# Wang-Ruocheng/QuanONet

Measured on AMD Instinct MI355X. Metric: train samples/sec (circuit-evals/sec alongside), QuanONet Q=5 Net40-2-20-2 Advection, higher is better.
Workload: dtype f64

## Files before the change

### quanonet_amd/csrc/hea_inst.hip

```cpp
#include "hea_device.hpp"
#include "hea_zyz.hpp"
#include "hea_qsweep.hpp"

#ifndef QHEA_N
#error "compile with -DQHEA_N=<qubits>"
#endif
#define QHEA_CAT_(a, b) a##b
#define QHEA_CAT(a, b) QHEA_CAT_(a, b)

namespace qhea {

void QHEA_CAT(launch_fwd_, QHEA_N)(dim3 grid, hipStream_t st, const FwdArgs& a) {
    hipLaunchKernelGGL(fwd_kernel<QHEA_N>, grid, dim3(kWaves * 64), 0, st, a.runs, a.B, a.E, a.cs, a.gates, a.gates_bytes, a.off,
                       a.co, a.diag, a.pauli, a.out, a.state_out, a.bias);
}
void QHEA_CAT(launch_bwd_, QHEA_N)(dim3 grid, hipStream_t st, const BwdArgs& a) {
#if QHEA_N == 8 || QHEA_N == 9
    if (a.dense) {
        hipLaunchKernelGGL((bwd_kernel<QHEA_N, 2>), grid, dim3(kWaves * 64), 0, st, a.runs, a.B, a.E, a.blk, a.cs, a.gates,
                           a.gates_bytes, a.off, a.co, a.diag, a.pauli, a.g, a.state_in, a.y, a.bias, a.inv_bt, a.out,
                           a.grad_x, a.partial);
        return;
    }
#endif
// ... 15 lines not shown
                       a.partial, DepthArgs{mrec, ms});
}

void QHEA_CAT(launch_bwd_qubit_, QHEA_N)(dim3 grid, hipStream_t st, const BwdArgs& a, const QubitArgs& q) {
#if QHEA_N >= 7
#if QHEA_N == 8 || QHEA_N == 9
    if (a.dense) {
        hipLaunchKernelGGL((bwd_kernel<QHEA_N, 2, QubitArgs>), grid, dim3(kWaves * 64), 0, st, a.runs, a.B, a.E, a.blk, a.cs, a.gates,
                           a.gates_bytes, a.off, a.co, a.diag, a.pauli, a.g, a.state_in, a.y, a.bias, a.inv_bt, a.out,
                           a.grad_x, a.partial, q);
        return;
    }
#endif
    hipLaunchKernelGGL((bwd_kernel<QHEA_N, 1, QubitArgs>), grid, dim3(kWaves * 64), 0, st, a.runs, a.B, a.E, a.blk, a.cs, a.gates,
                       a.gates_bytes, a.off, a.co, a.diag, a.pauli, a.g, a.state_in, a.y, a.bias, a.inv_bt, a.out, a.grad_x,
                       a.partial, q);
#else
    (void)grid; (void)st; (void)a; (void)q;
#endif
}

void QHEA_CAT(launch_bwd_pair_, QHEA_N)(dim3 grid, hipStream_t st, const BwdArgs& a) {
#if QHEA_N <= 5
    if (a.tri == 1) {
        hipLaunchKernelGGL(bwd_tri_kernel<QHEA_N>, grid, dim3(128 + 64 * kSigmaWaves), 0, st, a.runs, a.B, a.E, a.blk, a.cs, a.gates,
                           a.gates_bytes, a.off, a.co, a.diag, a.pauli, a.g, a.state_in, a.y, a.bias, a.inv_bt, a.out,
                           a.grad_x, a.partial, a.status);
        return;
    }
    hipLaunchKernelGGL(bwd_pair_kernel<QHEA_N>, grid, dim3(128), 0, st, a.runs, a.B, a.E, a.blk, a.cs, a.gates,
                       a.gates_bytes, a.off, a.co, a.diag, a.pauli, a.g, a.state_in, a.y, a.bias, a.inv_bt, a.out, a.grad_x,
                       a.partial, a.status);
#else
    (void)grid; (void)st; (void)a;
#endif
}

#if QHEA_N <= 5
void QHEA_CAT(launch_fwd_zyz_, QHEA_N)(dim3 grid, size_t dyn_lds, hipStream_t st, const ZFwdArgs& a) {
    hipLaunchKernelGGL(fwd_zyz_kernel<QHEA_N>, grid, dim3((kZFwdWaves + kFwdHelpers) * 64), dyn_lds, st, a);
}
void QHEA_CAT(launch_bwd_ztri_, QHEA_N)(dim3 grid, size_t dyn_lds, hipStream_t st, const ZBwdArgs& a, const char* mrec) {
    if (grid.y > 1) {
        const ZBwdArgsM am{a, mrec};
        if (a.pipes == 2) hipLaunchKernelGGL((bwd_ztri_kernel<QHEA_N, 2, ZBwdArgsM>), grid, dim3(2 * 64 * kZPipeWaves), dyn_lds, st, am);
        else hipLaunchKernelGGL((bwd_ztri_kernel<QHEA_N, 1, ZBwdArgsM>), grid, dim3(64 * kZPipeWaves), dyn_lds, st, am);
        return;
    }
    if (a.pipes == 2) hipLaunchKernelGGL((bwd_ztri_kernel<QHEA_N, 2>), grid, dim3(2 * 64 * kZPipeWaves), dyn_lds, st, a);
    else hipLaunchKernelGGL((bwd_ztri_kernel<QHEA_N, 1>), grid, dim3(64 * kZPipeWaves), dyn_lds, st, a);
}
void QHEA_CAT(launch_fwd_zshared_, QHEA_N)(dim3 grid, size_t dyn_lds, hipStream_t st, const ZFwdArgs& a) {
    hipLaunchKernelGGL(fwd_zshared_kernel<QHEA_N>, grid, dim3(kZPWaves * 64), dyn_lds, st, a);
}
void QHEA_CAT(launch_bwd_zpacked_, QHEA_N)(dim3 grid, size_t dyn_lds, hipStream_t st, const ZBwdArgs& a, const char* mrec) {
    if (grid.y > 1) hipLaunchKernelGGL((bwd_zpacked_kernel<QHEA_N, ZBwdArgsM>), grid, dim3(kZPWaves * 64), dyn_lds, st, ZBwdArgsM{a, mrec});
    else hipLaunchKernelGGL(bwd_zpacked_kernel<QHEA_N>, grid, dim3(kZPWaves * 64), dyn_lds, st, a);
}
#if QHEA_N == 5
void launch_fwd_split_5(dim3 grid, size_t dyn_lds, hipStream_t st, const ZFwdArgs& a) {
    hipLaunchKernelGGL(fwd_split_kernel<5>, grid, dim3((kSplitWaves + kSplitHelpers) * 64), dyn_lds, st, a);
}
void launch_bwd_zquad_5(dim3 grid, size_t dyn_lds, hipStream_t st, const ZBwdArgs& a, const char* mrec) {
    if (grid.y > 1) hipLaunchKernelGGL((bwd_zquad_kernel<kPairRing, kZSigma, ZBwdArgsM>), grid, dim3(64 * (4 + kZSigma)), dyn_lds, st, ZBwdArgsM{a, mrec});
    else hipLaunchKernelGGL((bwd_zquad_kernel<kPairRing, kZSigma>), grid, dim3(64 * (4 + kZSigma)), dyn_lds, st, a);
}
void launch_bwd_zsnap_5(dim3 grid, size_t dyn_lds, hipStream_t st, const ZBwdArgs& a) {
    hipLaunchKernelGGL((bwd_zsnap_kernel<kZSnapRing>), grid, dim3(64 * (4 + 2 * kZSigma)), dyn_lds, st, a);
}
#endif
#elif QHEA_N <= 5
void QHEA_CAT(launch_fwd_zyz_, QHEA_N)(dim3, size_t, hipStream_t, const ZFwdArgs&) {}
void QHEA_CAT(launch_bwd_ztri_, QHEA_N)(dim3, size_t, hipStream_t, const ZBwdArgs&, const char*) {}
void QHEA_CAT(launch_bwd_zpacked_, QHEA_N)(dim3, size_t, hipStream_t, const ZBwdArgs&, const char*) {}
void QHEA_CAT(launch_fwd_zshared_, QHEA_N)(dim3, size_t, hipStream_t, const ZFwdArgs&) {}
#if QHEA_N == 5
void launch_fwd_split_5(dim3, size_t, hipStream_t, const ZFwdArgs&) {}
void launch_bwd_zquad_5(dim3, size_t, hipStream_t, const ZBwdArgs&, const char*) {}
void launch_bwd_zsnap_5(dim3, size_t, hipStream_t, const ZBwdArgs&) {}
#endif
#endif

}
```

### quanonet_amd/csrc/hea_zyz.hpp

```cpp
#pragma once
#include "hea_device.hpp"
#include "hea_sincos.hpp"

namespace qhea {

constexpr int kRecBytes = 1024;
constexpr int kRecRy = 512;
constexpr int kZCsBytes = 20480;

__host__ __device__ inline long zyz_cs_row(int n, long E) { return E + 2 * n; }
__host__ __device__ inline bool zyz_eligible(int n, long E) {
    return n >= 2 && n <= 5 && (long)(64 >> n) * zyz_cs_row(n, E) * 16 <= kZCsBytes;
}
__host__ __device__ inline int zyz_layer_count(const Runs& r, int n) {
    long L = 0;
    for (int i = 0; i < r.nruns; ++i) L += (long)r.count[i] * ((r.enc[i] + n - 1) / n + r.ld[i]);
    return (int)L;
}

struct AngleSrc {
    const double* x;
    EncDesc enc;
    long m_rows = 0, m_params = 0;
};
// ... 129 lines not shown
        const int lc = l < 0 ? 0 : (l > L ? L : l);
        dma_record(rsrc, lds0 + (unsigned)(l & (kSlots - 1)) * kRecBytes, lane16, (unsigned)lc * kRecBytes);
    }
    __device__ __forceinline__ char* buf(int l) const { return ring + (l & (kSlots - 1)) * kRecBytes; }
    __device__ __forceinline__ double2 rd_diag(int l) const { return *reinterpret_cast<const double2*>(buf(l) + dgoff); }
    template <int Q>
    __device__ __forceinline__ double2 rd_ry(int l) const { return *reinterpret_cast<const double2*>(buf(l) + voff[Q]); }
    __device__ __forceinline__ void rd_all_ry(int l) { static_for<0, N>([&](auto q) { ry[decltype(q)::value] = rd_ry<decltype(q)::value>(l); }); }

    template <int D>
    __device__ __forceinline__ void prime(int l0) {
#pragma unroll
        for (int i = 0; i < kDist; ++i) issue(l0 + i * D);
        wait_vmcnt<kDist - 1>();
        dg = rd_diag(l0);
        rd_all_ry(l0);
    }
    template <int D>
    __device__ __forceinline__ void begin(int l) {
        issue(l + kDist * D);
        wait_vmcnt<kDist - 1>();
    }
};

template <int N>
__device__ __forceinline__ void zyz_forward(double (&re)[1], double (&im)[1], const Runs& runs, LayerStream<N>& ls,
                                            const double2* __restrict__ csrow, int E, int lane, int klow, int ring_fwd) {
    re[0] = klow == 0 ? 1.0 : 0.0;
    im[0] = 0.0;
    int l = 0, col = 0;
    ls.template prime<1>(0);
    double2 nxt[N];
    auto prefetch = [&](int c) {
        static_for<0, N>([&](auto q) {
            constexpr int Q = decltype(q)::value;
            const int e = c + Q;
            nxt[Q] = csrow[e < E ? e : (E > 0 ? E - 1 : 0)];
        });
    };
    if (E > 0) prefetch(0);
    for (int ri = 0; ri < runs.nruns; ++ri) {
        const int ne = runs.enc[ri], nld = runs.ld[ri];
        for (int rep = 0; rep < runs.count[ri]; ++rep) {
            for (int j0 = 0; j0 < ne; j0 += N) {
                const int m = (ne - j0) < N ? (ne - j0) : N;
                ls.template begin<1>(l);
                apply_phase<false>(re[0], im[0], ls.dg);
                ls.dg = ls.rd_diag(l + 1);
                for_gates_below<N>(m, [&](auto q) {
                    constexpr int Q = decltype(q)::value;
                    apply_enc<N, Q, false>(re, im, nxt[Q]);
                });
                prefetch(col + j0 + m);
                ls.rd_all_ry(l + 1);
                ++l;
            }
            col += ne;
            for (int s = 0; s < nld; ++s) {
                ls.template begin<1>(l);
                apply_phase<false>(re[0], im[0], ls.dg);
                ls.dg = ls.rd_diag(l + 1);
                static_for<0, N>([&](auto q) {
                    constexpr int Q = decltype(q)::value;
                    apply_ry<Q, false>(re[0], im[0], ls.ry[Q]);
                    ls.ry[Q] = ls.template rd_ry<Q>(l + 1);
                });
                re[0] = lane_gather(re[0], ring_fwd);
                im[0] = lane_gather(im[0], ring_fwd);
                ++l;
            }
        }
    }
    apply_phase<false>(re[0], im[0], ls.dg);
}

template <int K> using CtSlot = std::integral_constant<int, K>;
struct RtSlot { int b; };
template <class T> struct is_ct_slot : std::false_type {};
template <int K> struct is_ct_slot<CtSlot<K>> : std::true_type {};
constexpr int kBSlots = 4, kBDist = 2;
constexpr int kPadRecs = 9;
constexpr int kBlockRingBytes = kBSlots * 3 * kRecBytes;

template <int N, int LD, bool SHARED = false>
struct BlockStream {
    static constexpr int RPB = 1 + LD;
    bool loader = true;
    u32x4 rsrc;
    char* ring;
    unsigned lds0, lane16, a_dg;
    unsigned a_ry[N];
    double2 dg[RPB];
    double2 ry[LD][N];
    double2 cs[N];

    __device__ __forceinline__ void init(const char* rec0, int nrec , char* ring_wave, int lane, int klow) {
        const unsigned long long base = reinterpret_cast<unsigned long long>(rec0) - (unsigned long long)kPadRecs * kRecBytes;
        rsrc = u32x4{(unsigned)base, (unsigned)(base >> 32) & 0xffffu, (unsigned)((nrec + 2 * kPadRecs) * kRecBytes), 0x00020000u};
        ring = ring_wave;
        lds0 = (unsigned)(unsigned long long)(__attribute__((address_space(3))) char*)ring_wave;
        lane16 = (unsigned)lane * 16u;
        a_dg = (unsigned)klow * 16u;
        static_for<0, N>([&](auto q) {
            constexpr int Q = decltype(q)::value;
            a_ry[Q] = kRecRy + Q * 32 + (Q == 4 ? 1u : (((unsigned)lane >> Q) & 1u)) * 16u;
        });
    }
    __device__ __forceinline__ void issue(int b) const {
        const unsigned slot = lds0 + (unsigned)(b & (kBSlots - 1)) * (RPB * kRecBytes);
        const unsigned soff = (unsigned)((b * RPB + kPadRecs) * kRecBytes);
        dma_records<RPB>(rsrc, slot, lane16, soff);
    }
    __device__ __forceinline__ const char* slot(int b) const { return ring + (b & (kBSlots - 1)) * (RPB * kRecBytes); }
    template <int D, int K>
    static constexpr int slot_off(CtSlot<K>) { return ((K + D) & (kBSlots - 1)) * (RPB * kRecBytes); }
    template <int D>
    static __device__ __forceinline__ int slot_off(RtSlot s) { return ((s.b + D) & (kBSlots - 1)) * (RPB * kRecBytes); }
    template <int D, class SL>
    __device__ __forceinline__ const char* slot_rel(SL s) const { return ring + slot_off<D>(s); }
    template <int D, class SL>
    __device__ __forceinline__ void ahead_rel(SL s, int b) const {
        if (!SHARED || loader)
            dma_records<RPB>(rsrc, lds0 + (unsigned)slot_off<D>(s), lane16, (unsigned)(((b + D) * RPB + kPadRecs) * kRecBytes));
    }
    __device__ __forceinline__ void landed() const {
        if (!SHARED || loader) wait_vmcnt<(kBDist - 1) * RPB>();
        if constexpr (SHARED) __syncthreads();
    }
    __device__ __forceinline__ void landed_late() const {
        if (!SHARED || loader) wait_vmcnt<kBDist * RPB>();
        if constexpr (SHARED) __syncthreads();
    }
    template <int D>
    __device__ __forceinline__ void ahead(int b) const { if (!SHARED || loader) issue(b + (kBDist + 1) * D); }
    template <int D>
    __device__ __forceinline__ void step(int b) const {
        ahead<D>(b);
        if (!SHARED || loader) wait_vmcnt<kBDist * RPB>();
        if constexpr (SHARED) __syncthreads();
    }
    template <int D>
    __device__ __forceinline__ void prime(int b0, bool drain) const {
        if (!SHARED || loader) {
            if (drain) wait_vmcnt<0>();
        }
        if constexpr (SHARED) { if (drain) __syncthreads(); }
        if (!SHARED || loader) {
#pragma unroll
            for (int i = 0; i <= kBDist; ++i) issue(b0 + i * D);
            wait_vmcnt<kBDist * RPB>();
        }
        if constexpr (SHARED) __syncthreads();
    }
    static __device__ __forceinline__ double2 rd(const char* p, unsigned off) { return *reinterpret_cast<const double2*>(p + off); }
    __device__ __forceinline__ void load_records(const char* sl) {
#pragma unroll
        for (int i = 0; i < RPB; ++i) dg[i] = rd(sl, i * kRecBytes + a_dg);
#pragma unroll
        for (int s = 0; s < LD; ++s)
            static_for<0, N>([&](auto q) { ry[s][decltype(q)::value] = rd(sl, (1 + s) * kRecBytes + a_ry[decltype(q)::value]); });
    }
    __device__ __forceinline__ void load_cs(const double2* __restrict__ csrow, int c0) {
        const double2* p = csrow + c0;
        static_for<0, N>([&](auto q) { cs[decltype(q)::value] = p[decltype(q)::value]; });
    }
};
// ... 93 lines not shown
    }
}
template <int Q>
__device__ __forceinline__ double2 cs32_packed(const double2* chunk ) {
    if constexpr (Q == 4) { const double2 t = chunk[2 * Q]; return make_double2(t.y, t.x); }
    else return chunk[2 * Q + 1];
}

template <bool HALVES>
__device__ __forceinline__ void swap_dup(double x, double& A, double& B) {
    double y;
    asm("" : "=v"(y) : "0"(x));
    const unsigned lo = (unsigned)__double2loint(x), hi = (unsigned)__double2hiint(x);
    const unsigned lo2 = (unsigned)__double2loint(y), hi2 = (unsigned)__double2hiint(y);
    if constexpr (HALVES) {
        const auto l = __builtin_amdgcn_permlane32_swap(lo, lo2, false, false);
        const auto h = __builtin_amdgcn_permlane32_swap(hi, hi2, false, false);
        A = __hiloint2double((int)h[0], (int)l[0]); B = __hiloint2double((int)h[1], (int)l[1]);
    } else {
        const auto l = __builtin_amdgcn_permlane16_swap(lo, lo2, false, false);
        const auto h = __builtin_amdgcn_permlane16_swap(hi, hi2, false, false);
        A = __hiloint2double((int)h[0], (int)l[0]); B = __hiloint2double((int)h[1], (int)l[1]);
    }
}
__device__ __forceinline__ void split_phase(double& x, const double2& d ) {
    double A, B;
    swap_dup<true>(x, A, B);
    x = d.y * A + d.x * B;
}
template <int Q>
__device__ __forceinline__ void split_ry(double& x, const double2& u) {
    if constexpr (Q == 4) {
        double A, B;
        swap_dup<false>(x, A, B);
        x = u.x * A + u.y * B;
    } else {
        const double own = u.x * x;
        x = fma(u.y, xchg<(1 << Q)>(x), own);
    }
}
struct SplitCoef { double2 dg; double t[4]; double2 g4; };
template <int Q>
__device__ __forceinline__ void split_ry_tan(double& x, double t) {
    static_assert(Q < 4, "wire 4 keeps the swap form");
    x = fma(t, xchg<(1 << Q)>(x), x);
}
__device__ __forceinline__ void split_gates(double& x, const LayerCoef<5>& c) {
    static_for<0, 5>([&](auto q) { split_ry<decltype(q)::value>(x, c.g[decltype(q)::value]); });
}
__device__ __forceinline__ void split_gates(double& x, const SplitCoef& c) {
    static_for<0, 4>([&](auto q) { split_ry_tan<decltype(q)::value>(x, c.t[decltype(q)::value]); });
    split_ry<4>(x, c.g4);
}

template <int LD>
struct SplitStream : BlockStream<5, LD, false> {
    using Base = BlockStream<5, LD, false>;
    static constexpr int RPB = 1 + LD;
    unsigned a_cs[5];
    __device__ __forceinline__ void init_split(const char* srec0, int nrec, char* ring_wave, int lane) {
        Base::init(srec0, nrec, ring_wave, lane, lane & 31);
        this->a_dg = (unsigned)(lane & 31) * 24u + (unsigned)(lane >> 5) * 8u;
        static_for<0, 5>([&](auto q) {
            constexpr int Q = decltype(q)::value;
            const unsigned bit = ((unsigned)lane >> Q) & 1u;
            this->a_ry[Q] = Q == 4 ? kSRecRy + 64 + bit * 16u : kSRecRy + Q * 16 + bit * 8u;
            a_cs[Q] = Q * 32 + (Q == 4 ? (1u - bit) : bit) * 16u;
        });
    }
    static __device__ __forceinline__ double2 rd8(const char* p, unsigned off) {
        const double* q = reinterpret_cast<const double*>(p + off);
        return make_double2(q[0], q[1]);
    }
    template <bool DAG = false>
    __device__ __forceinline__ void read_ansatz(SplitCoef& c, const char* sl, int rec, unsigned a_diag) const {
        c.dg = rd8(sl, rec * kRecBytes + a_diag);
        static_for<0, 4>([&](auto q) {
            constexpr int Q = decltype(q)::value;
            c.t[Q] = *reinterpret_cast<const double*>(sl + rec * kRecBytes + (this->a_ry[Q] ^ (DAG ? 8u : 0u)));
        });
        c.g4 = Base::rd(sl, rec * kRecBytes + this->a_ry[4]);
    }
};

constexpr int kSnapBytes = 1024;
template <int LD, bool SNAP = false>
__device__ __forceinline__ double zsplit_forward(SplitStream<LD>& bs, const char* csrow, int nblocks, int lane, int ring_fwd,
                                                 char* snap_base = nullptr, unsigned snap_off = 0) {
    double x = lane == 0 ? 1.0 : 0.0;
    bs.template prime<1>(0, false);
    const char* cs_b = csrow;
    LayerCoef<5> ce;
    SplitCoef ca, cb;
    ce.dg = bs.rd8(bs.slot(0), bs.a_dg);
    static_for<0, 5>([&](auto q) { ce.g[decltype(q)::value] = bs.rd(cs_b, bs.a_cs[decltype(q)::value]); });
    auto read_layer = [&](SplitCoef& c, const char* sl, int rec) {
        bs.read_ansatz(c, sl, rec, bs.a_dg);
        __builtin_amdgcn_sched_barrier(0);
    };
    auto read_chunk = [&](const char* nx, int kb) {
        ce.dg = bs.rd8(nx, bs.a_dg);
        const char* cn = cs_b + (kb + 1) * (5 * 32);
        static_for<0, 5>([&](auto q) { ce.g[decltype(q)::value] = bs.rd(cn, bs.a_cs[decltype(q)::value]); });
        __builtin_amdgcn_sched_barrier(0);
    };
    auto layer = [&](const auto& c, bool ring, int pt) {
        split_phase(x, c.dg);
        split_gates(x, c);
        if constexpr (SNAP) {
            if (ring) {
                typedef __attribute__((address_space(1))) double gdouble;
                *(gdouble*)(snap_base + (size_t)(unsigned)pt * kSnapBytes + snap_off) = x;
            }
        }
        __builtin_amdgcn_sched_barrier(0);
        if (ring) x = lane_gather(x, ring_fwd);
    };
    auto block = [&](auto sl, int b, int kb) {
        const char* cur = bs.template slot_rel<0>(sl);
        const char* nx = bs.template slot_rel<1>(sl);
        read_layer(ca, cur, 1);
        layer(ce, false, 0);
        if constexpr (LD == 2) {
            read_layer(cb, cur, 2);
            layer(ca, true, 2 * b);
            bs.template ahead_rel<kBDist + 1>(sl, b);
            __builtin_amdgcn_sched_barrier(0);
            bs.landed_late();
            read_chunk(nx, kb);
            layer(cb, true, 2 * b + 1);
        } else {
            bs.landed();
            read_chunk(nx, kb);
            layer(ca, true, b);
            bs.template ahead_rel<kBDist + 1>(sl, b);
            __builtin_amdgcn_sched_barrier(0);
        }
    };
    int b = 0;
    for (; b + kBSlots <= nblocks; b += kBSlots) {
        block(CtSlot<0>{}, b, 0);
        block(CtSlot<1>{}, b + 1, 1);
        block(CtSlot<2>{}, b + 2, 2);
        block(CtSlot<3>{}, b + 3, 3);
        cs_b += kBSlots * (5 * 32);
    }
    for (; b < nblocks; ++b) {
        block(RtSlot{b}, b, 0);
        cs_b += 5 * 32;
    }
    split_phase(x, ce.dg);
    return x;
}

struct ZFwdArgs {
    Runs runs; long B; int E; const char* rec; int rec_bytes; int L; AngleSrc src; double off, co;
    const double* diag; int pauli; double* out; double* state_out; const double* bias;
    int fast_ld, nblocks;
    const char* srec;
};
struct MemberStride {
    long rows;
    long params;
    long grad;
    long ws;
};
template <class T>
__host__ __device__ __forceinline__ T* member_ptr(T* p, long bytes) {
    return p ? reinterpret_cast<T*>(reinterpret_cast<typename std::conditional<std::is_const<T>::value, const char, char>::type*>(p) + bytes) : p;
}
struct ZBwdArgs {
    Runs runs; long B; int E; int blk; const char* rec; int rec_bytes; int L; AngleSrc src; double off, co;
    const double* diag; int pauli; const double* g; const double* state_in; const double* y; const double* bias;
    double inv_bt; double* out; double* grad_x; double* partial; int* status;
    int fast_ld, nblocks;
    const char* srec;
    int pipes;
    MemberStride ms;
    char* snap = nullptr;
};
struct ZBwdArgsM : ZBwdArgs {
    const char* mrec;
};
struct MemberRec {
    double scale;
    double off, co;
    double lr;
    const double* diag;
    int pauli;
    int nq;
    int depth[2];
};
constexpr int kMemberRecOffset = 64;
static_assert(kMemberRecOffset + sizeof(MemberRec) <= 256, "MemberRec lives in the slice's 256-byte header");
template <class T>
__device__ __forceinline__ T* uniform_ptr(T* p) {
    const unsigned long long v = reinterpret_cast<unsigned long long>(p);
    const unsigned lo = (unsigned)__builtin_amdgcn_readfirstlane((int)(unsigned)v);
    const unsigned hi = (unsigned)__builtin_amdgcn_readfirstlane((int)(unsigned)(v >> 32));
    return reinterpret_cast<T*>(((unsigned long long)hi << 32) | lo);
}
template <class A> __device__ __forceinline__ long zm_ws(const A& a) { return (long)blockIdx.y * a.ms.ws; }
__device__ __forceinline__ const char* zm_rec(const ZBwdArgs& a) { return a.rec; }
__device__ __forceinline__ const char* zm_srec(const ZBwdArgs& a) { return a.srec; }
__device__ __forceinline__ double* zm_out(const ZBwdArgs& a) { return a.out; }
__device__ __forceinline__ double* zm_gx(const ZBwdArgs& a) { return a.grad_x; }
__device__ __forceinline__ double* zm_part(const ZBwdArgs& a) { return a.partial; }
__device__ __forceinline__ const double* zm_y(const ZBwdArgs& a) { return a.y; }
__device__ __forceinline__ const double* zm_bias(const ZBwdArgs& a) { return a.bias; }
__device__ __forceinline__ const char* zm_rec(const ZBwdArgsM& a) { return uniform_ptr(member_ptr(a.rec, zm_ws(a))); }
__device__ __forceinline__ const char* zm_srec(const ZBwdArgsM& a) { return uniform_ptr(member_ptr(a.srec, zm_ws(a))); }
__device__ __forceinline__ double* zm_out(const ZBwdArgsM& a) { return member_ptr(a.out, zm_ws(a)); }
__device__ __forceinline__ double* zm_gx(const ZBwdArgsM& a) { return member_ptr(a.grad_x, zm_ws(a)); }
__device__ __forceinline__ double* zm_part(const ZBwdArgsM& a) { return member_ptr(a.partial, zm_ws(a)); }
__device__ __forceinline__ const double* zm_y(const ZBwdArgsM& a) { return member_ptr(a.y, (long)blockIdx.y * a.ms.rows * (long)sizeof(double)); }
__device__ __forceinline__ const double* zm_bias(const ZBwdArgsM& a) { return member_ptr(a.bias, (long)blockIdx.y * a.ms.params * (long)sizeof(double)); }
typedef const __attribute__((address_space(4))) MemberRec* ConstMemberRec;
__device__ __forceinline__ ConstMemberRec zm_mr(const ZBwdArgsM& a) {
    return (ConstMemberRec)uniform_ptr(member_ptr(reinterpret_cast<const MemberRec*>(a.mrec), zm_ws(a)));
}
__device__ __forceinline__ double zm_off(const ZBwdArgs& a) { return a.off; }
// ... 621 lines not shown
            acc3[3 * Q + 2] = flip_sign(lm.x * pv.y - lm.y * pv.x, m);
        });
    };
    auto store_sums = [&](double (&acc3)[C::KW], int sub) {
        const int vi = butterfly_sum<C::KW>(acc3, lane);
        if (butterfly_owner<C::KW>(lane)) {
            if constexpr (SNAP) __hip_atomic_fetch_add(&row_lds[sub * C::KW + vi], acc3[0], __ATOMIC_RELAXED, __HIP_MEMORY_SCOPE_WORKGROUP);
            else store_through(&part_w[(long)sub * C::KW + vi], acc3[0]);
        }
    };
    const int LDr = a.fast_ld, nsteps = a.nblocks * LDr;
    const int slot_off = zquad_slot_offset<RING>(LDr, a.nblocks);
    const unsigned snap_lds = (unsigned)(unsigned long long)(__attribute__((address_space(3))) char*)(psi_ring[0]);
    int cur = 0;
    const int vs = sample_slot(lane), ax_slot = vs < 3 * N ? vs : 3 * N - 1;
    const int gx_src1 = sample_slot_lane(vs + 1, lane >> 5) * 4, gx_src2 = sample_slot_lane(vs + 2, lane >> 5) * 4;
    const long bs = wave * C::SPW + (lane >> 5);
    const bool gx_lane = (lane & 1) == 0 && vs < 3 * N && vs % 3 == 0 && bs < a.B;
    double* __restrict__ gx_w = zm_gx(a) + bs * E + vs / 3;
    auto fetch_snap = [&](int t, int sl) {
        asm volatile("s_mov_b32 m0, %0\n\ts_nop 0\n\tbuffer_load_dwordx4 %1, %2, %3 offen sc1 lds"
                     :: "s"(snap_lds + (unsigned)sl * kSnapBytes), "v"((unsigned)lane * 16u), "s"(snap_rsrc),
                        "s"((unsigned)(nsteps - 1 - t) * kSnapBytes) : "memory", "m0");
    };
    auto draw = [&]() {
        int v = 0;
        if (lane == 0) v = __hip_atomic_fetch_add(next, 1, __ATOMIC_RELAXED, __HIP_MEMORY_SCOPE_WORKGROUP);
        return v;
    };
    int mine = __builtin_amdgcn_readfirstlane(draw());
    __hip_atomic_store(&cursor[me], mine, __ATOMIC_RELEASE, __HIP_MEMORY_SCOPE_WORKGROUP);
    int after_v = draw();
    if constexpr (SNAP) {
        if (mine < nsteps) {
#pragma unroll
            for (int i = 0; i < NPROD; ++i) pair_wait_ge(&prod[i], 1, abort_flag, seen_c[i]);
            fetch_snap(mine, 0);
        }
    }
    auto sigma_step = [&](auto chunk_c) {
        constexpr bool CHUNK = decltype(chunk_c)::value;
        const int t = mine;
        const int j = LDr == 2 ? (t >> 1) : t;
        const int sub = a.blk - 1 - t, bl = a.nblocks - 1 - j;
#pragma unroll
        for (int i = 0; i < NPROD; ++i) pair_wait_ge(&prod[i], t + 1, abort_flag, seen_c[i]);
        if constexpr (SNAP) wait_vmcnt<0>();
        const double2* slot = SNAP ? psi_ring[cur] : psi_ring[(t + slot_off) & (RING - 1)];
        const double2 pv = slot[lane];
        double2 qv[N];
        static_for<0, N>([&](auto q) { qv[decltype(q)::value] = slot[lane ^ (1 << decltype(q)::value)]; });
        const double2 lm = lam_ring[(t + slot_off) & (RING - 1)][lane];
        double ax = 0.0;
        if constexpr (CHUNK) ax = axis_ring[(bl & (kAxisRing - 1)) * (3 * N) + ax_slot];
        if (lane == 0) __hip_atomic_store(&cursor[me], after_v, __ATOMIC_RELEASE, __HIP_MEMORY_SCOPE_WORKGROUP);
        mine = __builtin_amdgcn_readfirstlane(after_v);
        after_v = draw();
        if constexpr (SNAP) {
            cur ^= 1;
            if (mine < nsteps) fetch_snap(mine, cur);
        }
        double acc3[C::KW];
        products(acc3, pv, qv, lm);
        if constexpr (CHUNK) {
            sample_butterfly_sum16(acc3, lane);
            const double pr = ax * acc3[0];
            const double g = pr + lane_gather(pr, gx_src1) + lane_gather(pr, gx_src2);
            const double tot = pair_sum<32>(acc3[0]);
            if ((lane & 33) == 0) {
                if constexpr (SNAP) __hip_atomic_fetch_add(&row_lds[sub * C::KW + vs], tot, __ATOMIC_RELAXED, __HIP_MEMORY_SCOPE_WORKGROUP);
                else store_through(&part_w[(long)sub * C::KW + vs], tot);
            }
            if (gx_lane) store_through(&gx_w[bl * N], g);
        } else {
            store_sums(acc3, sub);
        }
    };
    while (mine < nsteps) {
        if (LDr == 1 || (mine & 1)) sigma_step(std::true_type{});
        else sigma_step(std::false_type{});
    }
}

template <int LD, int RING, int NSIG, bool SNAP = false, class A>
__device__ __forceinline__ void zquad_chain(const A& a, int role , int smp, int lane, bool valid, long b,
                                            const char* cs_tables, char* my_ring, double2 (*psi_ring)[64], double2 (*lam_ring)[64],
                                            double2* psi_final, ZQSync* sync, double* axis_ring, char* snap = nullptr) {
    constexpr int N = 5;
    __builtin_amdgcn_s_setprio(3);
    const int E = a.E, k = lane & 31, p = lane >> 5;
    const int ring_fwd = ring_source<N>(lane, false);
    const int ring_rev = ring_source<N>(lane, true);
    const unsigned mask4 = lane_sign_mask<4>(lane);
    SplitStream<LD> ss;
    ss.init_split(zm_srec(a), a.L + 1, my_ring, lane);
    const char* row = cs_tables + (smp * (int)zyz_cs_row(N, E) + N) * 32;
    const int slot_idx = (((smp << 5) | k) << 1) | p;
    int seen[NSIG], safe = 0;
#pragma unroll
    for (int w = 0; w < NSIG; ++w) seen[w] = 0;
    double x;
    if constexpr (SNAP) {
        x = zsplit_forward<LD, true>(ss, row, a.nblocks, lane, ring_fwd, snap, (unsigned)slot_idx * 8u);
        reinterpret_cast<double*>(psi_final)[slot_idx] = x;
        handoff_release();
    } else if (role == 0) {
        if (a.state_in) x = a.state_in[(((b << N) + k) << 1) | p];
        else x = zsplit_forward<LD>(ss, row, a.nblocks, lane, ring_fwd);
        reinterpret_cast<double*>(psi_final)[slot_idx] = x;
        handoff_release();
        if (lane == 0) __hip_atomic_store(&sync->ready[smp], 1, __ATOMIC_RELAXED, __HIP_MEMORY_SCOPE_WORKGROUP);
    }
    if (SNAP || role == 1) {
        int seen_ready = 0;
        if (!SNAP) pair_wait_ge(&sync->ready[smp], 1, &sync->abort, seen_ready);
        const double2 f = psi_final[(smp << 5) | k];
        const double h = ham_weight<N>(k, zm_off(a), zm_co(a), zm_diag(a));
        double v[1] = {h * (f.x * f.x + f.y * f.y)};
        lane_reduce<1, 5>(v, lane);
        const double pred = v[0] + (zm_bias(a) ? zm_bias(a)[0] : 0.0);
        if (zm_out(a) && valid && lane == 0) zm_out(a)[b] = pred;
        double gb = zm_y(a) ? 2.0 * (pred - zm_y(a)[b]) * a.inv_bt : a.g[b];
        if (!valid) gb = 0.0;
        x = gb * h * (p ? f.y : f.x);
    }
    const int nb = a.nblocks;
    double* ring_lane = reinterpret_cast<double*>(role == 0 ? psi_ring : lam_ring) + slot_idx;
    double* ring_pass = ring_lane;
    const int slot_off = zquad_slot_offset<RING>(LD, nb);
    int* prod = role == 0 ? &sync->psi_prod[smp] : &sync->lam_prod[smp];
    int step = 0;
    auto publish_data = [&](auto sl, auto sub) {
        wait_slot_free<NSIG>(sync->cursor, step - RING + 1, &sync->abort, seen, safe);
        if constexpr (LD == 2 && is_ct_slot<decltype(sl)>::value)
            ring_pass[(2 * (kBSlots - 1 - decltype(sl)::value) + decltype(sub)::value) * 128] = x;
        else
            ring_lane[((step + slot_off) & (RING - 1)) * 128] = x;
        ++step;
    };
    auto publish_flag = [&]() {
        handoff_release();
        __hip_atomic_store(prod, step, __ATOMIC_RELAXED, __HIP_MEMORY_SCOPE_WORKGROUP);
    };
    const unsigned a_dgd = (unsigned)k * 24u + (unsigned)(1 - p) * 8u;
    ss.template prime<-1>(nb, true);
    split_phase_dag(x, ss.rd8(ss.slot(nb), a_dgd));
    ss.template step<-1>(nb);
    const char* cs_b = row + (long)(nb - 1) * (N * 32);
    SplitCoef ct, cm;
    LayerCoef<N> c0;
    auto read_layer = [&](SplitCoef& c, const char* sl, int rec) {
        ss.template read_ansatz<true>(c, sl, rec, a_dgd);
        __builtin_amdgcn_sched_barrier(0);
    };
    auto read_chunk = [&](const char* sl, const char* chunk) {
        c0.dg = ss.rd8(sl, a_dgd);
        static_for<0, N>([&](auto q) { c0.g[decltype(q)::value] = ss.rd(chunk, ss.a_cs[decltype(q)::value]); });
        __builtin_amdgcn_sched_barrier(0);
    };
    auto undo_gates = [&](const auto& c) {
        split_gates_dag(x, c, mask4);
        __builtin_amdgcn_sched_barrier(0);
    };
    read_layer(ct, ss.slot(nb - 1), LD);
    static_assert(kAxisRing % kBSlots == 0, "a pass of the unrolled body stays within the axis ring");
    double* axis_lane = axis_ring + lane;
    double* axis_pass = axis_lane;
    typedef double vdouble2 __attribute__((ext_vector_type(2)));
    typedef __attribute__((address_space(3))) const vdouble2 lds_double2;
    unsigned cs_pass[N];
    auto read_chunk_pass = [&](const char* sl, auto k) {
        c0.dg = ss.rd8(sl, a_dgd);
        static_for<0, N>([&](auto q) {
            const vdouble2 v = *(lds_double2*)(unsigned long)(cs_pass[decltype(q)::value] + decltype(k)::value * (N * 32));
            c0.g[decltype(q)::value] = make_double2(v.x, v.y);
        });
        __builtin_amdgcn_sched_barrier(0);
    };
    auto block = [&](auto sl, int bl) {
        const char* cur = ss.template slot_rel<0>(sl);
        const char* nx = ss.template slot_rel<-1>(sl);
        auto chunk_coefs = [&]() {
            if constexpr (is_ct_slot<decltype(sl)>::value) read_chunk_pass(cur, sl);
            else read_chunk(cur, cs_b);
        };
        if (role == 1 && smp == 0 && lane < 3 * N) {
            const double ax = reinterpret_cast<const double*>(cur + kSRecRy)[lane];
            if constexpr (is_ct_slot<decltype(sl)>::value) axis_pass[decltype(sl)::value * (3 * N)] = ax;
            else axis_lane[(bl & (kAxisRing - 1)) * (3 * N)] = ax;
        }
        if constexpr (LD == 2) read_layer(cm, cur, 1);
        else chunk_coefs();
        x = lane_gather(x, ring_rev);
        ss.template ahead_rel<-(kBDist + 1)>(sl, bl);
        __builtin_amdgcn_sched_barrier(0);
        publish_data(sl, std::integral_constant<int, 0>{});
        undo_gates(ct);
        publish_flag();
        if constexpr (LD == 2) {
            chunk_coefs();
            split_phase_dag(x, ct.dg);
            x = lane_gather(x, ring_rev);
            __builtin_amdgcn_sched_barrier(0);
            publish_data(sl, std::integral_constant<int, 1>{});
            undo_gates(cm);
            publish_flag();
            split_phase_dag(x, cm.dg);
        } else {
            split_phase_dag(x, ct.dg);
        }
        ss.landed_late();
        read_layer(ct, nx, LD);
        undo_gates(c0);
        split_phase_dag(x, c0.dg);
    };
    int bl = nb - 1;
    for (; bl >= 0 && (bl & (kBSlots - 1)) != kBSlots - 1; --bl) {
        block(RtSlot{bl}, bl);
        cs_b -= N * 32;
    }
    for (; bl >= kBSlots - 1; bl -= kBSlots) {
        static_for<0, N>([&](auto q) {
            constexpr int Q = decltype(q)::value;
            cs_pass[Q] = (unsigned)(unsigned long long)(__attribute__((address_space(3))) const char*)(cs_b - (kBSlots - 1) * (N * 32)) + ss.a_cs[Q];
            asm("" : "+v"(cs_pass[Q]));
        });
        if constexpr (LD == 2) ring_pass = ring_lane + ((step + slot_off) & (RING - 1) & ~(2 * kBSlots - 1)) * 128;
        axis_pass = axis_lane + (bl & (kAxisRing - 1) & ~(kBSlots - 1)) * (3 * N);
        block(CtSlot<3>{}, bl);
        block(CtSlot<2>{}, bl - 1);
        block(CtSlot<1>{}, bl - 2);
        block(CtSlot<0>{}, bl - 3);
        cs_b -= kBSlots * (N * 32);
    }
}

template <int RING, int NSIG, class A = ZBwdArgs>
__global__ __launch_bounds__(64 * (4 + NSIG)) void bwd_zquad_kernel(A a) {
    constexpr int N = 5;
    using C = Cfg<N>;
    extern __shared__ __attribute__((aligned(16))) char dyn_lds[];
    char* fixed = dyn_lds;
    const int lane = threadIdx.x & 63;
    const int wv = __builtin_amdgcn_readfirstlane((int)(threadIdx.x >> 6));
    const int tid = (int)threadIdx.x;
    char* rec_ring = fixed;
    double2 (*psi_ring)[64] = reinterpret_cast<double2 (*)[64]>(fixed + 4 * kBlockRingBytes);
    double2 (*lam_ring)[64] = reinterpret_cast<double2 (*)[64]>(fixed + 4 * kBlockRingBytes + RING * 1024);
    double2* psi_final = reinterpret_cast<double2*>(fixed + 4 * kBlockRingBytes + 2 * RING * 1024);
    ZQSync& sync = *reinterpret_cast<ZQSync*>(fixed + 4 * kBlockRingBytes + 2 * RING * 1024 + 1024);
    static_assert(sizeof(ZQSync) <= 256, "reserved");
    double* axis_ring = reinterpret_cast<double*>(fixed + 4 * kBlockRingBytes + 2 * RING * 1024 + 1024 + 256);
    char* cs_tables = dyn_lds + zquad_fixed_lds(RING);
    const long wave = blockIdx.x;
    const int E = a.E;
    if (tid == 0) {
        sync.psi_prod[0] = sync.psi_prod[1] = sync.lam_prod[0] = sync.lam_prod[1] = 0;
        sync.ready[0] = sync.ready[1] = 0; sync.abort = 0;
        for (int w = 0; w < NSIG; ++w) sync.cursor[w] = 0;
        sync.next = 0;
    }
    fill_cs_split(reinterpret_cast<double4*>(cs_tables), zm_src(a), E, wave * C::SPW, a.B, C::SPW, tid, 64 * (4 + NSIG));
    __syncthreads();

    if (wv < 4) {
        const int role = wv >> 1, smp = wv & 1;
        const long b_raw = wave * C::SPW + smp;
        const bool valid = b_raw < a.B;
        const long b = valid ? b_raw : a.B - 1;
        char* my_ring = rec_ring + wv * kBlockRingBytes;
        if (a.fast_ld == 2) zquad_chain<2, RING, NSIG>(a, role, smp, lane, valid, b, cs_tables, my_ring, psi_ring, lam_ring, psi_final, &sync, axis_ring);
        else zquad_chain<1, RING, NSIG>(a, role, smp, lane, valid, b, cs_tables, my_ring, psi_ring, lam_ring, psi_final, &sync, axis_ring);
    } else {
        zsigma_walk<RING, 4>(a, lane, wv - 4, wave, psi_ring, lam_ring, axis_ring, &sync.psi_prod[0], &sync.abort, sync.cursor, &sync.next);
    }
    report_abort(&sync.abort, a.status, lane);
}

constexpr int kZSnapRing = 8;
__host__ __device__ constexpr size_t zsnap_fixed_lds(int ring) {
    return 2 * (size_t)kBlockRingBytes + (size_t)ring * 1024 + 1024 + 256 + (size_t)kAxisRing * 15 * sizeof(double) +
           (size_t)kZSigma * 2 * kSnapBytes;
}
template <int RING, class A = ZBwdArgs>
__global__ __launch_bounds__(64 * (4 + 2 * kZSigma)) __attribute__((amdgpu_waves_per_eu(4, 4))) void bwd_zsnap_kernel(A a) {
    constexpr int N = 5;
    using C = Cfg<N>;
    extern __shared__ __attribute__((aligned(16))) char dyn_lds[];
    const int lane = threadIdx.x & 63;
    const int wv = __builtin_amdgcn_readfirstlane((int)(threadIdx.x >> 6));
    const int tid = (int)threadIdx.x;
    const int grp = wv < 4 ? (wv >> 1) : (wv - 4) / kZSigma;
    char* fixed = dyn_lds + grp * (int)zsnap_fixed_lds(RING);
    char* rec_ring = fixed;
    double2 (*lam_ring)[64] = reinterpret_cast<double2 (*)[64]>(fixed + 2 * kBlockRingBytes);
    double2* psi_final = reinterpret_cast<double2*>(fixed + 2 * kBlockRingBytes + RING * 1024);
    ZQSync& sync = *reinterpret_cast<ZQSync*>(fixed + 2 * kBlockRingBytes + RING * 1024 + 1024);
    static_assert(sizeof(ZQSync) <= 256, "reserved");
    double* axis_ring = reinterpret_cast<double*>(fixed + 2 * kBlockRingBytes + RING * 1024 + 1024 + 256);
    char* snap_bufs = fixed + 2 * kBlockRingBytes + RING * 1024 + 1024 + 256 + kAxisRing * 15 * sizeof(double);
    char* lds_tables = dyn_lds + 2 * (int)zsnap_fixed_lds(RING);
    const int E = a.E;
    const int cs_bytes = (int)(C::SPW * zyz_cs_row(N, E) * 32);
    double* row_lds = reinterpret_cast<double*>(lds_tables + 2 * cs_bytes);
    const long wave = (long)blockIdx.x * 2 + grp;
    const int nsteps = a.nblocks * a.fast_ld;
    char* snap = a.snap + wave * (long)nsteps * kSnapBytes;
    if (tid < 2) {
        ZQSync& s = *reinterpret_cast<ZQSync*>(dyn_lds + tid * (int)zsnap_fixed_lds(RING) + 2 * kBlockRingBytes + RING * 1024 + 1024);
        s.psi_prod[0] = s.psi_prod[1] = s.lam_prod[0] = s.lam_prod[1] = 0;
        s.ready[0] = s.ready[1] = 0; s.abort = 0;
        for (int w = 0; w < kZSigma; ++w) s.cursor[w] = 0;
        s.next = 0;
    }
    for (int i = tid; i < a.blk * C::KW; i += 64 * (4 + 2 * kZSigma)) row_lds[i] = 0.0;
    fill_cs_split(reinterpret_cast<double4*>(lds_tables), a.src, E, (long)blockIdx.x * 2 * C::SPW, a.B, 2 * C::SPW, tid, 64 * (4 + 2 * kZSigma));
    __syncthreads();

    if (wv < 4) {
        const int smp = wv & 1;
        const long b_raw = wave * C::SPW + smp;
        const bool valid = b_raw < a.B;
        const long b = valid ? b_raw : a.B - 1;
        char* my_ring = rec_ring + smp * kBlockRingBytes;
        char* cs_tables = lds_tables + grp * cs_bytes;
        char* snap_u = uniform_ptr(snap);
        if (a.fast_ld == 2) zquad_chain<2, RING, kZSigma, true>(a, 1, smp, lane, valid, b, cs_tables, my_ring, lam_ring, lam_ring, psi_final, &sync, axis_ring, snap_u);
        else zquad_chain<1, RING, kZSigma, true>(a, 1, smp, lane, valid, b, cs_tables, my_ring, lam_ring, lam_ring, psi_final, &sync, axis_ring, snap_u);
    } else {
        const int me = (wv - 4) % kZSigma;
        const unsigned long long base = reinterpret_cast<unsigned long long>(uniform_ptr(snap));
        const u32x4 rsrc{(unsigned)base, (unsigned)(base >> 32) & 0xffffu, (unsigned)nsteps * kSnapBytes, 0x00020000u};
        double2 (*buf)[64] = reinterpret_cast<double2 (*)[64]>(snap_bufs + me * 2 * kSnapBytes);
        zsigma_walk<RING, 2, true>(a, lane, me, wave, buf, lam_ring, axis_ring, &sync.lam_prod[0], &sync.abort, sync.cursor, &sync.next,
                                   rsrc, row_lds);
    }
    report_abort(&sync.abort, a.status, lane);
    __syncthreads();
    double* __restrict__ row = zm_part(a) + (long)blockIdx.x * a.blk * C::KW;
    for (int i = tid; i < a.blk * C::KW; i += 64 * (4 + 2 * kZSigma)) store_through(&row[i], row_lds[i]);
}

constexpr int kZPWaves = 4;
__host__ __device__ inline long zp_cs_row(int n, long E) { return E + n; }
__host__ __device__ inline size_t zp_cs_bytes(int n, long E, int rows) { return ((size_t)rows * zp_cs_row(n, E) + n) * sizeof(double2); }

template <int Q>
__device__ __forceinline__ void ry_inv_with_inner(double& pr, double& pi, double& lr, double& li, const double2& u, int lane,
                                                  double& X, double& Y, double& Z) {
    const unsigned m = lane_sign_mask<Q>(lane);
    if constexpr (Q == 4) {
        const double qr = xchg<16>(pr), qi = xchg<16>(pi);
        X = lr * qi - li * qr;
        Y = flip_sign(-(lr * qr) - li * qi, m);
        Z = flip_sign(lr * pi - li * pr, m);
        apply_ry<4, true>(pr, pi, u);
        apply_ry<4, true>(lr, li, u);
    } else {
        const double qr = xchg<(1 << Q)>(pr), qi = xchg<(1 << Q)>(pi);
        X = lr * qi - li * qr;
        Y = flip_sign(-(lr * qr) - li * qi, m);
        Z = flip_sign(lr * pi - li * pr, m);
        pr = u.x * pr - u.y * qr;
        pi = u.x * pi - u.y * qi;
        apply_ry<Q, true>(lr, li, u);
    }
}
template <int N, int Q>
__device__ __forceinline__ void enc_inv_with_inner(double (&pr)[1], double (&pi)[1], double (&lr)[1], double (&li)[1],
                                                   const double2& cs, int lane, double& G) {
    if constexpr (Q == 4) {
        const double qr = xchg<16>(pr[0]), qi = xchg<16>(pi[0]);
        G = flip_sign(-(lr[0] * qr) - li[0] * qi, lane_sign_mask<Q>(lane));
        apply_ry<4, true>(pr[0], pi[0], cs);
        apply_ry<4, true>(lr[0], li[0], cs);
    } else {
        const double qr = xchg<(1 << Q)>(pr[0]), qi = xchg<(1 << Q)>(pi[0]);
        G = lr[0] * qi - li[0] * qr;
        const double nr = cs.x * pr[0] - cs.y * qi;
        pi[0] = cs.x * pi[0] + cs.y * qr;
        pr[0] = nr;
        apply_rx<N, Q>(lr, li, cs.x, -cs.y);
    }
}

template <int N, int LD, class A>
__device__ __forceinline__ void zpacked_body(const A& a, int wib, int lane, int klow, bool valid, long b, long wave,
                                             const double2* cs, char* wg_ring, double* comb ) {
    using C = Cfg<N>;
    const int E = a.E;
    const int ring_fwd = ring_source<N>(lane, false);
    const int ring_rev = ring_source<N>(lane, true);
    const double2* csrow = cs + (wib * C::SPW + (lane >> C::LB)) * (int)zp_cs_row(N, E) + N;
    BlockStream<N, LD, true> bs;
    bs.init(zm_rec(a), a.L + 1, wg_ring, lane, klow);
    bs.loader = wib == 0;

    double pr[1], pi[1], lr[1], li[1];
    if (a.state_in) {
        const double2 s0 = reinterpret_cast<const double2*>(a.state_in)[(b << N) + klow];
        pr[0] = s0.x; pi[0] = s0.y;
    } else {
        zyz_forward_fast<N, LD>(pr, pi, a.runs, bs, csrow, E, lane, klow, ring_fwd);
    }
    {
        double fr[1] = {pr[0]}, fi[1] = {pi[0]};
        basis_change<N, false>(fr, fi, zm_pauli(a), lane);
        const double h = ham_weight<N>(klow, zm_off(a), zm_co(a), zm_diag(a));
        double v[1] = {h * (fr[0] * fr[0] + fi[0] * fi[0])};
        lane_reduce<1, C::LB>(v, lane);
        const double pred = v[0] + (zm_bias(a) ? zm_bias(a)[0] : 0.0);
        if (zm_out(a) && valid && klow == 0) zm_out(a)[b] = pred;
        double gb = zm_y(a) ? 2.0 * (pred - zm_y(a)[b]) * a.inv_bt : a.g[b];
        if (!valid) gb = 0.0;
        lr[0] = gb * h * fr[0]; li[0] = gb * h * fi[0];
        basis_change<N, true>(lr, li, zm_pauli(a), lane);
    }

    const int nb = a.nblocks;
    bs.template prime<-1>(nb, true);
    {
        const double2 d = bs.rd(bs.slot(nb), bs.a_dg);
        apply_phase<true>(pr[0], pi[0], d);
// ... 158 lines not shown
```

Measured before the change: 14.52 million.

## Prefetch split-stream records before LDS setup and hoist turn loads in zsnap

The zsnap backward kernel now issues the first ring prefetches of the forward split stream before the cs-table fill and __syncthreads, so global loads overlap the LDS setup, and the forward pass then skips its own prime and only waits on vmcnt. The Hamiltonian weight, bias and target loads for the turn are also issued before the forward sweep rather than after it, which takes their latency off the critical path at the forward-to-backward turn. It also adds optional s_memtime stamps, compiled only under a macro, to profile the kernel phases. The trade-off is extra live registers and a reliance on an exact vmcnt count matching the number of prefetches issued.

```diff
diff --git a/quanonet_amd/csrc/hea_inst.hip b/quanonet_amd/csrc/hea_inst.hip
--- a/quanonet_amd/csrc/hea_inst.hip
+++ b/quanonet_amd/csrc/hea_inst.hip
@@ -121,3 +121,9 @@
 #endif
 
 }
+
+#if defined(QHEA_ZSNAP_STAMPS) && QHEA_N == 5
+extern "C" __attribute__((visibility("default"))) int qhea_zsnap_stamps_read(unsigned long long* out) {
+    return (int)hipMemcpyFromSymbol(out, HIP_SYMBOL(qhea::qhea_zsnap_stamps), sizeof(qhea::qhea_zsnap_stamps));
+}
+#endif
diff --git a/quanonet_amd/csrc/hea_zyz.hpp b/quanonet_amd/csrc/hea_zyz.hpp
--- a/quanonet_amd/csrc/hea_zyz.hpp
+++ b/quanonet_amd/csrc/hea_zyz.hpp
@@ -235,6 +235,19 @@
 constexpr int kPadRecs = 9;
 constexpr int kBlockRingBytes = kBSlots * 3 * kRecBytes;
 
+#ifdef QHEA_ZSNAP_STAMPS
+constexpr int kZStamps = 9;
+constexpr int kZStampLds = 2 * kBlockRingBytes + 8 * 1024 + 1024 + 128;
+static __device__ unsigned long long qhea_zsnap_stamps[kZStamps];
+__device__ __forceinline__ unsigned long long* zsnap_stamp_slots() {
+    extern __shared__ __attribute__((aligned(16))) char dyn_lds[];
+    return reinterpret_cast<unsigned long long*>(dyn_lds + kZStampLds);
+}
+#define QHEA_ZSTAMP(i) do { if (threadIdx.x == 0 && blockIdx.x == gridDim.x / 2) zsnap_stamp_slots()[i] = __builtin_amdgcn_s_memtime(); } while (0)
+#else
+#define QHEA_ZSTAMP(i) do {} while (0)
+#endif
+
 template <int N, int LD, bool SHARED = false>
 struct BlockStream {
     static constexpr int RPB = 1 + LD;
@@ -494,13 +507,21 @@
         c.g4 = Base::rd(sl, rec * kRecBytes + this->a_ry[4]);
     }
 };
+template <int LD>
+__device__ __forceinline__ void zsplit_prefetch(const char* srec0, int nrec, char* ring_wave, int lane) {
+    SplitStream<LD> ss;
+    ss.init_split(srec0, nrec, ring_wave, lane);
+#pragma unroll
+    for (int i = 0; i <= kBDist; ++i) ss.issue(i);
+}
 
 constexpr int kSnapBytes = 1024;
-template <int LD, bool SNAP = false>
+template <int LD, bool SNAP = false, bool PRIMED = false>
 __device__ __forceinline__ double zsplit_forward(SplitStream<LD>& bs, const char* csrow, int nblocks, int lane, int ring_fwd,
                                                  char* snap_base = nullptr, unsigned snap_off = 0) {
     double x = lane == 0 ? 1.0 : 0.0;
-    bs.template prime<1>(0, false);
+    if constexpr (PRIMED) wait_vmcnt<kBDist * SplitStream<LD>::RPB>();
+    else bs.template prime<1>(0, false);
     const char* cs_b = csrow;
     LayerCoef<5> ce;
     SplitCoef ca, cb;
@@ -549,6 +570,7 @@
             __builtin_amdgcn_sched_barrier(0);
         }
     };
+    if constexpr (SNAP) QHEA_ZSTAMP(2);
     int b = 0;
     for (; b + kBSlots <= nblocks; b += kBSlots) {
         block(CtSlot<0>{}, b, 0);
@@ -1336,6 +1358,16 @@
     }
 }
 
+struct TurnIn { double h, bias, yg; };
+template <class A>
+__device__ __forceinline__ TurnIn zturn_load(const A& a, int k, long b) {
+    TurnIn t;
+    t.h = ham_weight<5>(k, zm_off(a), zm_co(a), zm_diag(a));
+    t.bias = zm_bias(a) ? zm_bias(a)[0] : 0.0;
+    t.yg = zm_y(a) ? zm_y(a)[b] : a.g[b];
+    return t;
+}
+
 template <int LD, int RING, int NSIG, bool SNAP = false, class A>
 __device__ __forceinline__ void zquad_chain(const A& a, int role , int smp, int lane, bool valid, long b,
                                             const char* cs_tables, char* my_ring, double2 (*psi_ring)[64], double2 (*lam_ring)[64],
@@ -1353,9 +1385,12 @@
     int seen[NSIG], safe = 0;
 #pragma unroll
     for (int w = 0; w < NSIG; ++w) seen[w] = 0;
+    TurnIn turn{0.0, 0.0, 0.0};
+    if constexpr (SNAP) turn = zturn_load(a, k, b);
     double x;
     if constexpr (SNAP) {
-        x = zsplit_forward<LD, true>(ss, row, a.nblocks, lane, ring_fwd, snap, (unsigned)slot_idx * 8u);
+        x = zsplit_forward<LD, true, true>(ss, row, a.nblocks, lane, ring_fwd, snap, (unsigned)slot_idx * 8u);
+        QHEA_ZSTAMP(3);
         reinterpret_cast<double*>(psi_final)[slot_idx] = x;
         handoff_release();
     } else if (role == 0) {
@@ -1369,14 +1404,21 @@
         int seen_ready = 0;
         if (!SNAP) pair_wait_ge(&sync->ready[smp], 1, &sync->abort, seen_ready);
         const double2 f = psi_final[(smp << 5) | k];
-        const double h = ham_weight<N>(k, zm_off(a), zm_co(a), zm_diag(a));
+        double h;
+        if constexpr (SNAP) h = turn.h;
+        else h = ham_weight<N>(k, zm_off(a), zm_co(a), zm_diag(a));
         double v[1] = {h * (f.x * f.x + f.y * f.y)};
         lane_reduce<1, 5>(v, lane);
-        const double pred = v[0] + (zm_bias(a) ? zm_bias(a)[0] : 0.0);
+        double pred;
+        if constexpr (SNAP) pred = v[0] + turn.bias;
+        else pred = v[0] + (zm_bias(a) ? zm_bias(a)[0] : 0.0);
         if (zm_out(a) && valid && lane == 0) zm_out(a)[b] = pred;
-        double gb = zm_y(a) ? 2.0 * (pred - zm_y(a)[b]) * a.inv_bt : a.g[b];
+        double gb;
+        if constexpr (SNAP) gb = zm_y(a) ? 2.0 * (pred - turn.yg) * a.inv_bt : turn.yg;
+        else gb = zm_y(a) ? 2.0 * (pred - zm_y(a)[b]) * a.inv_bt : a.g[b];
         if (!valid) gb = 0.0;
         x = gb * h * (p ? f.y : f.x);
+        if constexpr (SNAP) QHEA_ZSTAMP(4);
     }
     const int nb = a.nblocks;
     double* ring_lane = reinterpret_cast<double*>(role == 0 ? psi_ring : lam_ring) + slot_idx;
@@ -1468,6 +1510,7 @@
         undo_gates(c0);
         split_phase_dag(x, c0.dg);
     };
+    if constexpr (SNAP) QHEA_ZSTAMP(5);
     int bl = nb - 1;
     for (; bl >= 0 && (bl & (kBSlots - 1)) != kBSlots - 1; --bl) {
         block(RtSlot{bl}, bl);
@@ -1487,6 +1530,7 @@
         block(CtSlot<0>{}, bl - 3);
         cs_b -= kBSlots * (N * 32);
     }
+    if constexpr (SNAP) QHEA_ZSTAMP(6);
 }
 
 template <int RING, int NSIG, class A = ZBwdArgs>
@@ -1544,6 +1588,11 @@
     const int lane = threadIdx.x & 63;
     const int wv = __builtin_amdgcn_readfirstlane((int)(threadIdx.x >> 6));
     const int tid = (int)threadIdx.x;
+    QHEA_ZSTAMP(0);
+#ifdef QHEA_ZSNAP_STAMPS
+    static_assert(kZStampLds == 2 * kBlockRingBytes + RING * 1024 + 1024 + 128 && sizeof(ZQSync) <= 128 &&
+                  kZStamps * sizeof(unsigned long long) <= 128, "the stamps sit in the spare half of group 0's sync block");
+#endif
     const int grp = wv < 4 ? (wv >> 1) : (wv - 4) / kZSigma;
     char* fixed = dyn_lds + grp * (int)zsnap_fixed_lds(RING);
     char* rec_ring = fixed;
@@ -1567,16 +1616,21 @@
         for (int w = 0; w < kZSigma; ++w) s.cursor[w] = 0;
         s.next = 0;
     }
+    const int smp = wv & 1;
+    const long b_raw = wave * C::SPW + smp;
+    const bool valid = b_raw < a.B;
+    const long b = valid ? b_raw : a.B - 1;
+    char* my_ring = rec_ring + smp * kBlockRingBytes;
+    if (wv < 4) {
+        if (a.fast_ld == 2) zsplit_prefetch<2>(zm_srec(a), a.L + 1, my_ring, lane);
+        else zsplit_prefetch<1>(zm_srec(a), a.L + 1, my_ring, lane);
+    }
     for (int i = tid; i < a.blk * C::KW; i += 64 * (4 + 2 * kZSigma)) row_lds[i] = 0.0;
     fill_cs_split(reinterpret_cast<double4*>(lds_tables), a.src, E, (long)blockIdx.x * 2 * C::SPW, a.B, 2 * C::SPW, tid, 64 * (4 + 2 * kZSigma));
     __syncthreads();
+    QHEA_ZSTAMP(1);
 
     if (wv < 4) {
-        const int smp = wv & 1;
-        const long b_raw = wave * C::SPW + smp;
-        const bool valid = b_raw < a.B;
-        const long b = valid ? b_raw : a.B - 1;
-        char* my_ring = rec_ring + smp * kBlockRingBytes;
         char* cs_tables = lds_tables + grp * cs_bytes;
         char* snap_u = uniform_ptr(snap);
         if (a.fast_ld == 2) zquad_chain<2, RING, kZSigma, true>(a, 1, smp, lane, valid, b, cs_tables, my_ring, lam_ring, lam_ring, psi_final, &sync, axis_ring, snap_u);
@@ -1591,8 +1645,15 @@
     }
     report_abort(&sync.abort, a.status, lane);
     __syncthreads();
+    QHEA_ZSTAMP(7);
     double* __restrict__ row = zm_part(a) + (long)blockIdx.x * a.blk * C::KW;
     for (int i = tid; i < a.blk * C::KW; i += 64 * (4 + 2 * kZSigma)) store_through(&row[i], row_lds[i]);
+#ifdef QHEA_ZSNAP_STAMPS
+    wait_vmcnt<0>();
+    QHEA_ZSTAMP(8);
+    if (tid == 0 && blockIdx.x == gridDim.x / 2)
+        for (int i = 0; i < kZStamps; ++i) qhea_zsnap_stamps[i] = zsnap_stamp_slots()[i];
+#endif
 }
 
 constexpr int kZPWaves = 4;
```

New measurement: 14.37 million. 0.99x the previous value.
